# DJjjjhao/FIRA-ICSE

Measured on AMD Instinct MI355X. Metric: training commits/sec (FIRA default config), higher is better.
Workload: dtype f32; 1 GPU; BASELINE configs[1]: FIRA training step (fwd+bwd+Adam, dropout 0.1/0.2), batch 32 commits/GPU, fp32, 650-node graphs (mean nnz 1066/graph), vocab 24650; global_batch=32, parallelism=dp1

## Files before the change

fira_icse_amd/_lib.py:

```python
from __future__ import annotations

import ctypes as C
import os

HERE = os.path.dirname(os.path.abspath(__file__))
LIB_PATH = os.environ.get("FIRA_HIP_LIB") or os.path.join(HERE, "libfira_hip.so")


class FiraError(RuntimeError):
    pass


class Dims(C.Structure):
    _fields_ = [("sou_len", C.c_int32), ("sub_len", C.c_int32), ("ast_len", C.c_int32), ("tar_len", C.c_int32),
                ("d_model", C.c_int32), ("n_head", C.c_int32), ("n_layer", C.c_int32), ("vocab", C.c_int32),
                ("ast_vocab", C.c_int32), ("d_ff", C.c_int32)]


class Batch(C.Structure):
    _fields_ = [("B", C.c_int32), ("nnz", C.c_int32), ("sou", C.c_void_p), ("tar", C.c_void_p), ("mark", C.c_void_p),
                ("ast_change", C.c_void_p), ("tar_label", C.c_void_p), ("sub_token", C.c_void_p),
                ("n_nodes", C.c_int32), ("node_rows", C.c_void_p), ("rowptr", C.c_void_p), ("col", C.c_void_p),
                ("val", C.c_void_p), ("n_code", C.c_int32), ("code_rows", C.c_void_p), ("code_mark", C.c_void_p),
                ("n_mem", C.c_int32), ("mem_rows", C.c_void_p), ("mem_dst", C.c_void_p), ("head_rows", C.c_void_p),
# ... 59 lines not shown
    "fira_combination_block_bwd": (_I, [_P, _I, _P, _P, _P, _P, _P, _P, _P, _P, _P, _I, _P, _P, _P, _P, _P, _P, _I, _P, _F, _U64, _U32, _U32, _I]),
    "fira_combination_block_bwd_part_floats": (_I, []),
    "fira_embed_gather_fwd": (_I, [_P, _I, _I, _P, _P, _P, _P, _I, _I]),
    "fira_embed_gather_bwd": (_I, [_P, _I, _I, _P, _P, _P, _I, _I, _I]),
    "fira_combination_fwd": (_I, [_P, _I, _P, _P, _P, _P, _F, _U64, _U32]),
    "fira_combination_bwd": (_I, [_P, _I, _P, _P, _P, _P, _P, _P, _F, _U64, _U32]),
    "fira_add_layernorm_fwd": (_I, [_P, _I, _P, _P, _P, _P, _P, _P, _F, _U64, _U32]),
    "fira_linear_presum_f32": (_I, [_P, _I, _I, _P, _I, _P, _P, _P, _P, _F, _U64, _U32]),
    "fira_ln_linear_f32": (_I, [_P, _I, _I, _P, _I, _P, _P, _P, _I, _I, _P, _P, _P, _P]),
    "fira_ln_bwd_linear_f32": (_I, [_P, _I, _I, _P, _P, _P, _P, _P, _P, _P, _P, _P, _P, _P, _P, _F, _U64, _U32]),
    "fira_linear_layernorm_bf16_fwd": (_I, [_P, _I, _P, _I, _P, _I, _P, _P, _P, _P, _P, _P, _P, _F, _U64, _U32]),
    "fira_add_layernorm_bwd": (_I, [_P, _I, _P, _P, _P, _P, _P, _P, _P, _P, _F, _U64, _U32]),
    "fira_dropout_mask": (_I, [_P, _U64, _U32, _L, _F, _P]),
    "fira_colsum_f32": (_I, [_P, _I, _I, _P, _I, _P]),
    "fira_attention_fwd": (_I, [_P, _I, _I, _I, _I, _P, _I, _P, _I, _P, _I, _P, _I, _I, _P, _I]),
    "fira_attention_bwd": (_I, [_P, _I, _I, _I, _I, _P, _I, _P, _I, _P, _I, _P, _I, _I, _P, _I, _P, _I,
                                _P, _I, _P, _I, _P, _I]),
    "fira_attention_fwd_ex": (_I, [_P, _I, _I, _I, _I, _P, _I, _P, _I, _P, _I, _P, _I, _I, _P, _I, _P, _I, _I, _P]),
    "fira_attention_bwd_ex": (_I, [_P, _I, _I, _I, _I, _P, _I, _P, _I, _P, _I, _P, _I, _I, _P, _I, _P, _I,
                                   _P, _I, _P, _I, _P, _I, _P, _I, _I, _P]),
    "fira_decode_attention": (_I, [_P, _I, _I, _I, _P, _I, _P, _I, _P, _I, _P, _P, _I, _I, _I, _I, _P, _P, _I, _P, _P, _P]),
    "fira_copy_score_fwd": (_I, [_P, _I, _I, _I, _P, _P, _P, _P, _P]),
    "fira_copy_score_bwd": (_I, [_P, _I, _I, _I, _P, _P, _P, _P, _P, _P, _P, _P]),
    "fira_head_loss": (_I, [_P, _I, _I, _I, _I, _P, _P, _I, _P, _P, _P, _P, _P, _P, _P, _I]),
    "fira_adam_step": (_I, [_P, _L, _P, _P, _P, _P, _F, _F, _F, _F, _I, _P]),
    "fira_adam_step_mb": (_I, [_P, _L, _P, _P, _P, _P, _P, _F, _F, _F, _F, _I, _P, _P]),
    "fira_inv_count": (_I, [_P, _P, _P]),
    "fira_adam_step_count": (_I, [_P, _L, _P, _P, _P, _P, _F, _F, _F, _F, _I, _P]),
    "fira_pack_stats": (_I, [_P, _P, _P, _P]),
    "fira_debug_chain": (_I, [_P, _I, _I, _P]),
    "fira_train_fwd_bwd": (_I, [_P, _DP, _BP, _P, _P, _P, _Z, _OP, _P, _P, _P]),
    "fira_train_step": (_I, [_P, _DP, _BP, _P, _P, _P, _Z, _OP, _P, _P, C.POINTER(AdamOpts)]),
    "fira_gemm_wgrad_panel": (_I, [_P, _I, _I, _I, _I, _P, _I, _P, _I, _P, _I, _P, _P, _Z]),
    "fira_ffn_fwd": (_I, [_P, _I, _I] + [_P] * 11 + [_F, _U64, _U32, _I]),
    "fira_ffn_bwd": (_I, [_P, _I, _I] + [_P] * 17 + [_F, _U64, _U32, _I]),
    "fira_head_topk": (_I, [_P, _I, _I, _I, _P, _P, _P, _P, _I, _P, _P, _I]),
    "fira_train_step_rows": (_I, [_P, _DP, _BP, _P, _P, _P, _Z, _OP, _P, _P, C.POINTER(AdamOpts), _P]),
    "fira_adam_rows_sync": (_I, [_P, _DP, _P, C.POINTER(AdamOpts), _P]),
    "fira_adam_rows_catchup": (_I, [_P, _DP, _P, C.POINTER(AdamOpts), _P, _I, _P, _I]),
    "fira_adam_rows_step": (_I, [_P, _DP, _P, _P, C.POINTER(AdamOpts), _P, _P, _P, _I]),
    "fira_train_step_begin_rows": (_I, [_P, _DP, _BP, _P, _P, _P, _Z, _OP, _P, _P, _P, C.POINTER(AdamOpts), _P]),
    "fira_train_step_end_rows": (_I, [_P, _P, C.POINTER(AdamOpts), _P, _P, _P]),
    "fira_grad_sqsum_scratch_bytes": (_Z, []),
    "fira_grad_sqsum": (_I, [_P, _L, _P, _P, _I, _P]),
    "fira_clip_finish": (_I, [_P, _P, _I, _P, _P, _F]),
    "fira_adam_step_clip": (_I, [_P, _L, _P, _P, _P, _P, _F, _F, _F, _F, _I, _P, _P, _P]),
# ... 109 lines not shown
```

fira_icse_amd/csrc/copyhead.hip:

```cpp
#include "engine.h"
#include "adam_rows.h"
#include <stdlib.h>
#include "epilogue.h"
#include "decode_row.h"

namespace fira {

constexpr int T_MAX = 32;

__device__ __forceinline__ float tanh_fast(float x) {
    const float e = __expf(2.0f * x);
    return 1.0f - __fdividef(2.0f, 1.0f + e);
}

__global__ __launch_bounds__(256) void copy_score_fwd_kernel(int T, int S, const float* __restrict__ src,
                                                             const float* __restrict__ tgt,
                                                             const float* __restrict__ w,
                                                             const float* __restrict__ bias,
                                                             float* __restrict__ score, int qpk,
                                                             const int32_t* __restrict__ mem_valid, int slots,
                                                             const int32_t* __restrict__ tar_label, int V,
                                                             const int32_t* __restrict__ t_off) {
    __shared__ __attribute__((aligned(16))) float sm_tgt[T_MAX * FIRA_D];
    __shared__ unsigned sm_mask;
// ... 13 lines not shown
    const float4 w4 = *reinterpret_cast<const float4*>(w + lane * 4);
    const float c = bias[0];
    const int j_end = min(S, (int)(blockIdx.x + 1) * slots);
    for (int j = blockIdx.x * slots + wave; j < j_end; j += 4) {
        if (mv && mv[j] == 0) {
            if (lane < Tb) score[((size_t)tb + lane) * S + j] = 0.f;
            continue;
        }
        const float4 s4 = *reinterpret_cast<const float4*>(src + ((size_t)b * S + j) * FIRA_D + lane * 4);
        for (int t = 0; t < Tb; ++t) {
            if (!((mask >> t) & 1u)) continue;
            const float4 x = *reinterpret_cast<const float4*>(&sm_tgt[t * FIRA_D + lane * 4]);
            float a = w4.x * tanh_fast(s4.x + x.x);
            a = fmaf(w4.y, tanh_fast(s4.y + x.y), a);
            a = fmaf(w4.z, tanh_fast(s4.z + x.z), a);
            a = fmaf(w4.w, tanh_fast(s4.w + x.w), a);
            a = wave_sum(a);
            if (lane == 0) score[((size_t)tb + t) * S + j] = a + c;
        }
    }
}

constexpr int COPY_KA = 8;
__global__ __launch_bounds__(256) void copy_score_bwd_kernel(int T, int S, const float* __restrict__ src,
                                                             const float* __restrict__ tgt,
                                                             const float* __restrict__ w,
                                                             const float* __restrict__ dscore,
                                                             float* __restrict__ dsrc, float* __restrict__ dtgt,
                                                             float* __restrict__ dw, float* __restrict__ dbias,
                                                             const int32_t* __restrict__ mem_valid, int slots,
                                                             float* __restrict__ part,
                                                             const int32_t* __restrict__ t_off) {
    constexpr int SLOTS_MAX = 16, SPW = SLOTS_MAX / 4;
    __shared__ __attribute__((aligned(16))) float sm_tgt[COPY_KA * FIRA_D];
    __shared__ float sm_dt[COPY_KA * FIRA_D];
    __shared__ float sm_dw[FIRA_D + 1];
    __shared__ float sm_g[T_MAX * SLOTS_MAX];
    __shared__ unsigned sm_mask;
    const int b = blockIdx.y, t0 = threadIdx.x, lane = t0 & 63, wave = t0 >> 6;
    const int j0 = blockIdx.x * slots, j_end = min(S, j0 + slots);
    const int tb = t_off ? t_off[b] : b * T;
    const int Tb = t_off ? t_off[b + 1] - tb : T;
    if (t0 == 0) sm_mask = 0u;
    __syncthreads();
    for (int i = t0; i < Tb * slots; i += 256) {
        const int t = i / slots, j = j0 + i % slots;
        float g = 0.f;
        if (j < j_end && !(mem_valid && mem_valid[(size_t)b * S + j] == 0)) g = dscore[((size_t)tb + t) * S + j];
        sm_g[t * SLOTS_MAX + i % slots] = g;
        if (g != 0.f) atomicOr(&sm_mask, 1u << t);
    }
    for (int i = t0; i < FIRA_D + 1; i += 256) sm_dw[i] = 0.f;
    __syncthreads();
    const unsigned mask = sm_mask;
    float* const my_part = part ? part + ((size_t)blockIdx.y * gridDim.x + blockIdx.x) * COPY_PART_STRIDE : nullptr;
    if (mask == 0u) {
        for (int j = j0 + wave; j < j_end; j += 4)
            *reinterpret_cast<float4*>(dsrc + ((size_t)b * S + j) * FIRA_D + lane * 4) = make_float4(0.f, 0.f, 0.f, 0.f);
        if (my_part)
            for (int i = t0; i < FIRA_D + 1; i += 256) my_part[i] = 0.f;
        return;
    }
    const float4 w4 = *reinterpret_cast<const float4*>(w + lane * 4);
    const float wv[4] = {w4.x, w4.y, w4.z, w4.w};
    float4 s4[SPW];
    float ds[SPW][4];
    bool live[SPW];
#pragma unroll
    for (int q = 0; q < SPW; ++q) {
        const int j = j0 + wave + 4 * q;
        live[q] = j < j_end && !(mem_valid && mem_valid[(size_t)b * S + min(j, S - 1)] == 0);
        s4[q] = live[q] ? *reinterpret_cast<const float4*>(src + ((size_t)b * S + j) * FIRA_D + lane * 4)
                        : make_float4(0.f, 0.f, 0.f, 0.f);
#pragma unroll
        for (int e = 0; e < 4; ++e) ds[q][e] = 0.f;
    }
    float dwa[4] = {0.f, 0.f, 0.f, 0.f};
    float dba = 0.f;
    unsigned rem = mask;
    while (rem) {
        int tl[COPY_KA], nk = 0;
#pragma unroll
        for (int k = 0; k < COPY_KA; ++k) {
            tl[k] = 0;
            if (rem) { tl[k] = __ffs(rem) - 1; rem &= rem - 1; nk = k + 1; }
        }
#pragma unroll
        for (int k = 0; k < COPY_KA; ++k)
            if (k < nk && t0 < FIRA_D / 4)
                reinterpret_cast<float4*>(sm_tgt)[k * (FIRA_D / 4) + t0] =
                    reinterpret_cast<const float4*>(tgt + ((size_t)tb + tl[k]) * FIRA_D)[t0];
        for (int i = t0; i < COPY_KA * FIRA_D; i += 256) sm_dt[i] = 0.f;
        __syncthreads();
        float dt[COPY_KA][4];
#pragma unroll
        for (int k = 0; k < COPY_KA; ++k)
#pragma unroll
            for (int e = 0; e < 4; ++e) dt[k][e] = 0.f;
#pragma unroll
        for (int q = 0; q < SPW; ++q) {
            if (!live[q]) continue;
            const int jj = wave + 4 * q;
#pragma unroll
            for (int k = 0; k < COPY_KA; ++k) {
                if (k < nk) {
                    const float g = sm_g[tl[k] * SLOTS_MAX + jj];
                    const float4 x = *reinterpret_cast<const float4*>(&sm_tgt[k * FIRA_D + lane * 4]);
                    const float th[4] = {tanh_fast(s4[q].x + x.x), tanh_fast(s4[q].y + x.y), tanh_fast(s4[q].z + x.z),
                                         tanh_fast(s4[q].w + x.w)};
#pragma unroll
                    for (int e = 0; e < 4; ++e) {
                        const float u = g * wv[e] * (1.f - th[e] * th[e]);
                        ds[q][e] += u;
                        dt[k][e] += u;
                        dwa[e] = fmaf(g, th[e], dwa[e]);
                    }
                    dba += g;
                }
            }
        }
#pragma unroll
        for (int k = 0; k < COPY_KA; ++k)
            if (k < nk) {
#pragma unroll
                for (int e = 0; e < 4; ++e) atomicAdd(&sm_dt[k * FIRA_D + lane * 4 + e], dt[k][e]);
            }
        __syncthreads();
#pragma unroll
        for (int k = 0; k < COPY_KA; ++k)
            if (k < nk) unsafeAtomicAdd(&dtgt[((size_t)tb + tl[k]) * FIRA_D + t0], sm_dt[k * FIRA_D + t0]);
        __syncthreads();
    }
#pragma unroll
    for (int q = 0; q < SPW; ++q) {
        const int j = j0 + wave + 4 * q;
        if (j < j_end)
            *reinterpret_cast<float4*>(dsrc + ((size_t)b * S + j) * FIRA_D + lane * 4) = make_float4(ds[q][0], ds[q][1], ds[q][2], ds[q][3]);
    }
#pragma unroll
    for (int e = 0; e < 4; ++e) atomicAdd(&sm_dw[lane * 4 + e], dwa[e]);
    if (lane == 0) atomicAdd(&sm_dw[FIRA_D], dba);
    __syncthreads();
    if (my_part) {
        for (int i = t0; i < FIRA_D + 1; i += 256) my_part[i] = sm_dw[i];
        return;
    }
    for (int i = t0; i < FIRA_D; i += 256) unsafeAtomicAdd(&dw[i], sm_dw[i]);
    if (t0 == 0) unsafeAtomicAdd(dbias, sm_dw[FIRA_D]);
}

__device__ __forceinline__ float block_max(float v, float* sm) {
    v = wave_max(v);
    __syncthreads();
    if ((threadIdx.x & 63) == 0) sm[threadIdx.x >> 6] = v;
    __syncthreads();
    return fmaxf(fmaxf(sm[0], sm[1]), fmaxf(sm[2], sm[3]));
}
__device__ __forceinline__ float block_sum(float v, float* sm) {
    v = wave_sum(v);
    __syncthreads();
    if ((threadIdx.x & 63) == 0) sm[threadIdx.x >> 6] = v;
    __syncthreads();
    return (sm[0] + sm[1]) + (sm[2] + sm[3]);
}
__device__ __forceinline__ void block_argmax(float& v, int& idx, float* smv, int* smi) {
#pragma unroll
    for (int o = 32; o > 0; o >>= 1) {
        const float ov = __shfl_xor(v, o, 64);
        const int oi = __shfl_xor(idx, o, 64);
        if (ov > v || (ov == v && oi < idx)) { v = ov; idx = oi; }
    }
// ... 554 lines not shown
    else
    hipLaunchKernelGGL(decode_dist_kernel, dim3(R), dim3(256), 0, s, V, S, logits, ldl, score, mem_valid, qpk,
                       gate_logits, dist, best_id, best_p);
    FIRA_CHECK_LAUNCH("decode_dist");
    return 0;
}

int copy_score_fwd_ex(hipStream_t s, int B, int T, int S, const float* src, const float* tgt, const float* w,
                      const float* bias, float* score, int qpk, const int32_t* mem_valid, const int32_t* tar_label,
                      int V, const int32_t* t_off) {
    ProfScope prof(s, PROF_COPY, 0.0);
    if (B <= 0) return 0;
    FIRA_REQUIRE(T <= T_MAX && qpk >= 1, "copy_score_fwd: T=%d > %d", T, T_MAX);
    const int slots = 8;
    hipLaunchKernelGGL(copy_score_fwd_kernel, dim3(cdiv(S, slots), B), dim3(256), 0, s, T, S, src, tgt, w, bias, score,
                       qpk, mem_valid, slots, tar_label, V, t_off);
    FIRA_CHECK_LAUNCH("copy_score_fwd");
    return 0;
}
int copy_score_fwd(hipStream_t s, int B, int T, int S, const float* src, const float* tgt, const float* w,
                   const float* bias, float* score) {
    return copy_score_fwd_ex(s, B, T, S, src, tgt, w, bias, score, 1, nullptr, nullptr, 0, nullptr);
}
int copy_score_bwd_blocks(int B, int S) { return B > 0 ? cdiv(S, 16) * B : 0; }
int copy_score_bwd_ex(hipStream_t s, int B, int T, int S, const float* src, const float* tgt, const float* w,
                      const float* dscore, float* dsrc, float* dtgt, float* dw, float* dbias, const int32_t* mem_valid,
                      float* part, const int32_t* t_off) {
    ProfScope prof(s, PROF_COPY, 0.0);
    if (B <= 0) return 0;
    FIRA_REQUIRE(T <= T_MAX, "copy_score_bwd: T=%d > %d", T, T_MAX);
    const int slots = 16;
    hipLaunchKernelGGL(copy_score_bwd_kernel, dim3(cdiv(S, slots), B), dim3(256), 0, s, T, S, src, tgt, w, dscore, dsrc,
                       dtgt, dw, dbias, mem_valid, slots, part, t_off);
    FIRA_CHECK_LAUNCH("copy_score_bwd");
    return 0;
}
int copy_score_bwd(hipStream_t s, int B, int T, int S, const float* src, const float* tgt, const float* w,
                   const float* dscore, float* dsrc, float* dtgt, float* dw, float* dbias) {
    return copy_score_bwd_ex(s, B, T, S, src, tgt, w, dscore, dsrc, dtgt, dw, dbias, nullptr, nullptr, nullptr);
}
int head_loss(hipStream_t s, int BT, int T, int V, int S, const int32_t* compact_row, float* logits, int ldl,
              float* score, const int32_t* mem_valid, float* gate_logits, const int32_t* tar_label, float* loss_sum,
              int32_t* n_tok, int32_t* argmax_out, int want_grad, const int32_t* row_bt) {
    ProfScope prof(s, PROF_HEAD, 0.0);
    if (BT <= 0) return 0;
    const bool reg = (V % 2 == 0) && (V / 2 <= 256 * HL_PAIRS) && (ldl % 2 == 0) && ((uintptr_t)logits % 8 == 0);
    if (reg && !argmax_out)
        hipLaunchKernelGGL(head_loss_train_kernel, dim3(BT), dim3(256), 0, s, T, V, S, compact_row, logits, ldl, score,
                           mem_valid, gate_logits, tar_label, loss_sum, n_tok, want_grad, row_bt);
    else if (reg)
        hipLaunchKernelGGL(head_loss_kernel<true>, dim3(BT), dim3(256), 0, s, T, V, S, compact_row, logits, ldl, score,
                           mem_valid, gate_logits, tar_label, loss_sum, n_tok, argmax_out, want_grad, row_bt);
    else
        hipLaunchKernelGGL(head_loss_kernel<false>, dim3(BT), dim3(256), 0, s, T, V, S, compact_row, logits, ldl, score,
                           mem_valid, gate_logits, tar_label, loss_sum, n_tok, argmax_out, want_grad, row_bt);
    FIRA_CHECK_LAUNCH("head_loss");
    return 0;
}
int adam_step(hipStream_t s, int64_t n, float* p, const float* g, float* m, float* v, float lr, float beta1,
              float beta2, float eps, int step, const float* scale_ptr, int scale_is_count) {
    ProfScope prof(s, PROF_ADAM, 0.0);
    if (n <= 0) return 0;
// ... 62 lines not shown
    const int grid = std::min(cdiv(total, 4), 256 * 8);
    hipLaunchKernelGGL(adam_rows_catchup_kernel, dim3(grid), dim3(256), 0, s, tb, l, beta1, beta2, eps, to,
                       adam_rows_hist(lr, beta1, beta2, to), 0.0f);
    FIRA_CHECK_LAUNCH("adam_rows_catchup");
    return 0;
}
int inv_count(hipStream_t s, const int32_t* n_tok, float* out) {
    hipLaunchKernelGGL(inv_count_kernel, dim3(1), dim3(1), 0, s, n_tok, out);
    FIRA_CHECK_LAUNCH("inv_count");
    return 0;
}

}

extern "C" {
int fira_copy_score_fwd(void* stream, int B, int T, int S, const float* src, const float* tgt, const float* w,
                        const float* bias, float* score) {
    return fira::copy_score_fwd((hipStream_t)stream, B, T, S, src, tgt, w, bias, score);
}
int fira_copy_score_bwd(void* stream, int B, int T, int S, const float* src, const float* tgt, const float* w,
                        const float* dscore, float* dsrc, float* dtgt, float* dw, float* dbias) {
    return fira::copy_score_bwd((hipStream_t)stream, B, T, S, src, tgt, w, dscore, dsrc, dtgt, dw, dbias);
}
int fira_head_loss(void* stream, int BT, int T, int V, int S, const int32_t* compact_row, float* logits, int ldl,
                   float* score, const int32_t* mem_valid, float* gate_logits, const int32_t* tar_label,
                   float* loss_sum, int32_t* n_tok, int32_t* argmax_out, int want_grad) {
    return fira::head_loss((hipStream_t)stream, BT, T, V, S, compact_row, logits, ldl, score, mem_valid, gate_logits,
                           tar_label, loss_sum, n_tok, argmax_out, want_grad);
}
int fira_adam_step_mb(void* stream, int64_t n, float* p, const float* g0, const float* g1, float* m, float* v, float lr,
                      float beta1, float beta2, float eps, int step, const int32_t* n_tok0, const int32_t* n_tok1) {
    FIRA_REQUIRE(p && g0 && m && v && n_tok0 && step >= 1, "fira_adam_step_mb: bad argument");
    return fira::adam_step_mb((hipStream_t)stream, n, p, g0, g1, m, v, lr, beta1, beta2, eps, step, n_tok0, n_tok1);
}
int fira_inv_count(void* stream, const int32_t* n_tok, float* out) {
    return fira::inv_count((hipStream_t)stream, n_tok, out);
}
int fira_adam_step(void* stream, int64_t n, float* p, const float* g, float* m, float* v, float lr, float beta1,
                   float beta2, float eps, int step, const float* inv_scale_ntok) {
    return fira::adam_step((hipStream_t)stream, n, p, g, m, v, lr, beta1, beta2, eps, step, inv_scale_ntok, 0);
}
int fira_adam_step_count(void* stream, int64_t n, float* p, const float* g, float* m, float* v, float lr, float beta1,
                         float beta2, float eps, int step, const float* count) {
    FIRA_REQUIRE(p && g && m && v && count && step >= 1, "fira_adam_step_count: bad argument");
    return fira::adam_step((hipStream_t)stream, n, p, g, m, v, lr, beta1, beta2, eps, step, count, 1);
}
// ... 8 lines not shown
```

fira_icse_amd/csrc/engine.h:

```cpp
#pragma once
#include "common.h"
#include <string>
#include <vector>

namespace fira {

int gemm_f32(hipStream_t s, int tA, int tB, int M, int N, int K, const float* A, int lda, const float* B, int ldb,
             float* C, int ldc, const float* bias, int flags, int splitk);
int gemm_f32_ex(hipStream_t s, int tA, int tB, int M, int N, int K, const float* A, int lda, const float* B, int ldb,
                float* C, int ldc, const float* bias, int flags, int splitk, float* colsum,
                const int32_t* c_rows = nullptr, const float* relu_mask = nullptr);
int gemm_bf16_ex(hipStream_t s, int tA, int tB, int M, int N, int K, const float* A, int lda, const float* B, int ldb,
                 float* C, int ldc, const float* bias, int flags, int splitk, float* colsum,
                 const int32_t* c_rows = nullptr, const float* relu_mask = nullptr);
struct ShadowEntry { int64_t offset; int rows, cols, pitch_t; int64_t offset_t; };
constexpr int SHADOW_MAX = 64;
struct ShadowTable {
    int n = 0;
    int64_t wbt_elems = 0;
    int tile_start[SHADOW_MAX + 1] = {0};
    ShadowEntry e[SHADOW_MAX];
};
int weight_shadows(hipStream_t s, const ShadowTable& tab, const float* P, uint16_t* Wb, uint16_t* WbT);
int gemm_bf16_wb_ex(hipStream_t s, int M, int N, int K, const float* A, int lda, const uint16_t* Bb, int ldb, float* C,
// ... 160 lines not shown
                     const float* V, int ldv, const int32_t* key_valid, float* O, int ldo, int kb, int kvb, int qpk,
                     const float* Knew = nullptr, const float* Vnew = nullptr, int ldn = 0, float* Kc_out = nullptr,
                     float* Vc_out = nullptr, const int32_t* k_off = nullptr);
int decode_self_block(hipStream_t s, int BR, int Tk, int T, const float* qkv, float* Kc, float* Vc, const int32_t* hist,
                      const float* WoT, const float* bo, const float* xres, const float* gamma, const float* beta,
                      const float* WqT, const float* bq, float* xa, float* qc);
int decode_attention_kv16(hipStream_t s, int BR, int H, int Tk, const float* Q, int ldq, const uint16_t* K, int ldk,
                          const uint16_t* V, int ldv, const int32_t* key_valid, float* O, int ldo, int kb, int kvb, int qpk,
                          const int32_t* k_off = nullptr);
int rows_to_bf16(hipStream_t s, int64_t n, const float* in, uint16_t* out);
int rows_from_bf16(hipStream_t s, int64_t n, const uint16_t* in, float* out);
int attention_bwd(hipStream_t s, int B, int H, int Tq, int Tk, const float* Q, int ldq, const float* K, int ldk,
                  const float* V, int ldv, const int32_t* key_valid, int causal, int q_pos0, const float* O, int ldo,
                  const float* dO, int lddo, float* dQ, int lddq, float* dK, int lddk, float* dV, int lddv,
                  const int32_t* q_off = nullptr, int self_kv = 0, int bf16 = 0, const int32_t* k_off = nullptr);
int copy_score_fwd(hipStream_t s, int B, int T, int S, const float* src, const float* tgt, const float* w,
                   const float* bias, float* score);
int copy_score_fwd_ex(hipStream_t s, int B, int T, int S, const float* src, const float* tgt, const float* w,
                      const float* bias, float* score, int qpk, const int32_t* mem_valid,
                      const int32_t* tar_label = nullptr, int V = 0,
                      const int32_t* t_off = nullptr);
int copy_score_bwd_ex(hipStream_t s, int B, int T, int S, const float* src, const float* tgt, const float* w,
                      const float* dscore, float* dsrc, float* dtgt, float* dw, float* dbias, const int32_t* mem_valid,
                      float* part = nullptr, const int32_t* t_off = nullptr);
int copy_score_bwd_blocks(int B, int S);
constexpr int COPY_PART_STRIDE = 264;
int decode_dist(hipStream_t s, int R, int V, int S, const float* logits, int ldl, const float* score,
                const int32_t* mem_valid, int qpk, const float* gate_logits, float* dist, int32_t* best_id,
                float* best_p, const float* x = nullptr, const float* wp = nullptr, const float* bp = nullptr);
int inv_count(hipStream_t s, const int32_t* n_tok, float* out);
int sample_dist(hipStream_t s, int R, int n_sample, int V, int S, const float* logits, int ldl, const float* score,
                const int32_t* mem_valid, const float* x, const float* wp, const float* bp, int T, int step,
                const int32_t* key, const uint64_t* seed_dev, float temperature, int top_k, float top_p, float* dist,
                int32_t* best_id, float* best_p);
int score_dist(hipStream_t s, int R, int n_cand, int V, int L, int S, const float* logits, int ldl, const float* score,
               const int32_t* mem_valid, const float* x, const float* wp, const float* bp, const int32_t* target,
               const int32_t* label, const int32_t* sou, const int32_t* sub, float* dist, float* p_word, float* p_entry,
               int32_t* entry, float* copy_share, float* p_label, int32_t* top_id, float* logp_word, float* logp_entry,
               float* logp_label);
int row_topk(hipStream_t s, int R, int V, int k, const float* logits, int ldl, int32_t* ids, float* vals);
int copy_score_bwd(hipStream_t s, int B, int T, int S, const float* src, const float* tgt, const float* w,
                   const float* dscore, float* dsrc, float* dtgt, float* dw, float* dbias);
int head_loss(hipStream_t s, int BT, int T, int V, int S, const int32_t* compact_row, float* logits, int ldl,
              float* score, const int32_t* mem_valid, float* gate_logits, const int32_t* tar_label, float* loss_sum,
              int32_t* n_tok, int32_t* argmax_out, int want_grad,
              const int32_t* row_bt = nullptr);
int adam_step(hipStream_t s, int64_t n, float* p, const float* g, float* m, float* v, float lr, float beta1,
              float beta2, float eps, int step, const float* scale_ptr, int scale_is_count = 0);
// ... 72 lines not shown
```

fira_icse_amd/csrc/engine.hip:

```cpp
#include "engine.h"
#include <hip/hip_ext.h>
#include "epilogue.h"
#include <stdlib.h>
#include <map>
#include <mutex>

namespace fira {

static int64_t shadow_wbt_elems(const Layout& L);

struct Arena {
    char* base;
    size_t used = 0;
    explicit Arena(void* b) : base((char*)b) {}
    template <typename T>
    T* get(size_t n) {
        size_t bytes = (n * sizeof(T) + 255) / 256 * 256;
        T* p = base ? (T*)(base + used) : nullptr;
        used += bytes;
        return p;
    }
    float* f(size_t n) { return get<float>(n); }
};

// ... 27 lines not shown
    std::vector<DecGrad> decg;
    float *vtab_all, *H, *mem, *mem_c, *src_c, *x0, *kv_all, *src, *tgt, *score, *gate, *dec_c, *logits;
    float *W21, *c21, *rsum;
    float *W21t;
    uint16_t *W21x = nullptr, *W21tx = nullptr;
    uint16_t *WcX = nullptr, *WcTX = nullptr;
    uint16_t* WkvX = nullptr;
    float* WkvT = nullptr;
    uint16_t* WkvTX = nullptr;
    uint16_t* WoutTX = nullptr;
    uint16_t *xh_planes = nullptr;
    float *WcT;
    float *dW21, *dc21;
    float *inv_ntok;
    float *dXa, *dXb, *dNB2, *dCB_a, *dvtab_all;
    float *zero_beg = nullptr, *zero_end = nullptr;
    uint16_t *wb = nullptr, *wbt = nullptr;
    uint16_t *w21b = nullptr, *w21bt = nullptr;
    float* red_buf = nullptr;
    size_t red_cap = 0;
    float* panel_scratch = nullptr;
    size_t panel_floats = 0;
    float *dmem_c, *dsrc, *dsrc_c, *dtgt, *dkv_all, *ddec, *ddec_c, *dT_a, *dT_c;

    size_t build(void* ws, const fira_dims& d, int B_, bool training) {
        Arena a(ws);
        B = B_; L = d.sou_len; S = d.sub_len; A = d.ast_len; T = d.tar_len; V = d.vocab; nl = d.n_layer; F = d.d_ff;
        N = L + S + A;
        NB = B * N; CB = B * L; MB = B * (L + S); TB = B * T;
        ldl = (V + 63) / 64 * 64;
        const size_t D = FIRA_D;
        pos_code = a.f((size_t)L * D);
        pos_tar = a.f((size_t)T * D);
        mem_valid = a.get<int32_t>((size_t)MB);
        tar_valid = a.get<int32_t>((size_t)TB);
        compact_row = a.get<int32_t>((size_t)TB);
        iota = a.get<int32_t>((size_t)TB);
        row_bt = a.get<int32_t>((size_t)TB);
        rows_c = a.get<int32_t>((size_t)TB);
        code_slot = a.get<int32_t>((size_t)NB);
        mem_slot = a.get<int32_t>((size_t)NB);
        mem_off = a.get<int32_t>((size_t)B + 1);
        mem_valid_c = a.get<int32_t>((size_t)MB);
        inv_ntok = a.f(64);
        {
            const Layout* lay = get_layout(&d);
// ... 39 lines not shown
            e.st_a = a.f((size_t)TB * 2); e.x_a = a.f((size_t)TB * D); e.qc = a.f((size_t)TB * D);
            e.ao2 = a.f((size_t)TB * D); e.s_c = a.f((size_t)TB * D); e.st_c = a.f((size_t)TB * 2);
            e.x_c = a.f((size_t)TB * D); e.h = a.f((size_t)TB * F); e.s_f = a.f((size_t)TB * D);
            e.st_f = a.f((size_t)TB * 2); e.x_f = a.f((size_t)TB * D);
        }
        src = a.f((size_t)MB * D); tgt = a.f((size_t)TB * D);
        score = a.f((size_t)TB * (L + S)); gate = a.f((size_t)TB * 2);
        dec_c = a.f((size_t)TB * D); logits = a.f((size_t)TB * ldl);
        if (training) {
            dXa = a.f((size_t)NB * D); dXb = a.f((size_t)NB * D); dNB2 = a.f((size_t)NB * D);
            dCB_a = a.f((size_t)CB * D);
            red_cap = (size_t)nl * ((size_t)cdiv(NB, 16) * 4 * D + (size_t)cdiv(CB, 16) * 2 * D)
                    + (size_t)3 * nl * cdiv(TB, 16) * 2 * D
                    + (size_t)nl * std::max((size_t)cdiv(CB, 16) * 4 * D, (size_t)comb_fused_bwd_parts() * 6 * D + 64)
                    + (size_t)cdiv(L + S, 16) * B * COPY_PART_STRIDE + 4096;
            red_buf = a.f(red_cap);
            panel_floats = (size_t)320 * 256 * 256;
            panel_scratch = a.f(panel_floats);
            zero_beg = (float*)a.get<char>(0);
            dvtab_all = a.f((size_t)4 * nl * D);
            dW21 = a.f((size_t)nl * D * D + (size_t)nl * D); dc21 = dW21 + (size_t)nl * D * D;
            dtgt = a.f((size_t)TB * D);
            ddec_c = a.f((size_t)TB * D);
            zero_end = (float*)a.get<char>(0);
            dmem_c = a.f((size_t)MB * D); dsrc = a.f((size_t)MB * D); dsrc_c = a.f((size_t)MB * D);
            dkv_all = a.f((size_t)MB * kvp);
            ddec = a.f((size_t)TB * D);
            dT_a = a.f((size_t)TB * D); dT_c = a.f((size_t)TB * D);
            encg.resize(nl);
            decg.resize(nl);
            for (int l = 0; l < nl; ++l) {
                EncGrad& g = encg[l];
                g.dY2 = a.f((size_t)NB * D); g.dYc = a.f((size_t)CB * D);
                g.dqk = a.f((size_t)CB * 2 * D);
                DecGrad& h = decg[l];
                h.dYf = a.f((size_t)TB * D); h.dh = a.f((size_t)TB * F); h.dYc = a.f((size_t)TB * D);
                h.dq = a.f((size_t)TB * D); h.dYs = a.f((size_t)TB * D); h.dqkv = a.f((size_t)TB * 3 * D);
            }
        }
        return a.used;
    }
};

#define TRY(x)                 \
    do {                       \
        if (int e__ = (x)) return e__; \
    } while (0)
// ... 863 lines not shown
    const bool so = side_on();
    hipStream_t ss = so ? side().aux : s;
    hipEvent_t ev_dfc = nullptr;
    if (c.ev_zero) TRY(main_wait(s, c.ev_zero, __LINE__));
    else TRY(zero(s, p.zero_beg, (size_t)((char*)p.zero_end - (char*)p.zero_beg)));
    if (R > 0) {
        if (so) TRY(aux_fork(s));
        if (c.wout_planes) TRY(dgrad_x3_splitk(ss, R, p.V, p.logits, p.ldl, p.WoutTX, p.ddec_c, D, g_dtype == 1));
        else
        TRY(gemm_any(ss, 0, 0, R, D, p.V, p.logits, p.ldl, c.P + L.wout, D, p.ddec_c, D, nullptr, FIRA_GEMM_ACCUM, 0,
                        nullptr));
        if (so) TRY(side_mark(&ev_dfc));
    }
    if (R > 0)
        TRY(linear_wgrad(s, R, p.V, D, p.logits, p.ldl, (c.rows != nullptr && rows == c.rows) ? p.dec_c : dec, D, G + L.wout,
                         G + L.bout, PANEL_VOCAB));
    if (g_dtype == 0) TRY(rank2_rows(s, c.Td, p.gate, c.P + L.wp, p.ddec));
    else TRY(linear_dgrad(s, c.Td, 2, D, p.gate, 2, c.P + L.wp, p.ddec, D, false));
    TRY(linear_wgrad_grouped(s, c.Td, 2, D, p.gate, 2, dec, D, G + L.wp, G + L.bp));
    {
        const int nb = copy_score_bwd_blocks(p.B, Sm);
        float* part = red().alloc((size_t)nb * COPY_PART_STRIDE);
        TRY(copy_score_bwd_ex(s, p.B, p.T, Sm, p.src, p.tgt, c.P + L.wres, p.score, p.dsrc, p.dtgt, G + L.wres, G + L.bres,
                              p.mem_valid, part, c.dec_off));
        if (part) {
            red().add(G + L.wres, part, D, nb, COPY_PART_STRIDE);
            red().add(G + L.bres, part + D, 1, nb, COPY_PART_STRIDE);
        }
    }
    TRY(linear_dgrad(s, c.Td, D, D, p.dtgt, D, c.P + L.wt, p.ddec, D, true));
    TRY(linear_wgrad_grouped(s, c.Td, D, D, p.dtgt, D, dec, D, G + L.wt, nullptr));
    TRY(rows_move(s, 0, Mc, D, p.dsrc_c, p.dsrc, bt.mem_dst, nullptr));
    if (so) TRY(aux_fork(s));
    TRY(linear_dgrad(ss, Mc, D, D, p.dsrc_c, D, c.P + L.ws, p.dmem_c, D, false));
    TRY(linear_wgrad_grouped(s, Mc, D, D, p.dsrc_c, D, p.mem_c, D, G + L.ws, nullptr, 8));
    if (R > 0) {
        if (ev_dfc) TRY(main_wait(s, ev_dfc, __LINE__));
        TRY(rows_scatter_add_idx(s, R, p.ddec_c, p.ddec, rows));
    }

    float *bx = p.ddec, *by = p.dT_a, *bz = p.dT_c;
    constexpr int DEC_WGRAD_EVERY = 3;
    const int dec_every = p.nl % DEC_WGRAD_EVERY != 0 ? 0 : DEC_WGRAD_EVERY;
    {
    ProfScope prof_region(s, PROF_DEC_REGION, 0.0);
    TRY(lanes_fork(c));
    auto aux_fork_all = [&]() -> int { return c.n_lanes > 1 ? lanes_fork_to(c, side().aux) : aux_fork(s); };
// ... 934 lines not shown
```

fira_icse_amd/ops.py:

```python
from __future__ import annotations

import dataclasses

import torch

from . import _lib
from ._lib import check, cur_stream, ptr


def _f32(t):
    assert t.is_cuda and t.dtype == torch.float32 and t.is_contiguous(), "expected a contiguous fp32 CUDA tensor"
    return t


def _i32(t):
    assert t.is_cuda and t.dtype == torch.int32 and t.is_contiguous(), "expected a contiguous int32 CUDA tensor"
    return t


def gemm(A, B, *, transA=False, transB=True, bias=None, relu=False, out=None, accumulate=False, splitk=1,
         tile=0, dtype="f32"):
    for t in (A, B):
        assert t.is_cuda and t.dtype == torch.float32 and t.dim() == 2 and t.stride(1) == 1
    M, K = (A.shape[1], A.shape[0]) if transA else A.shape
# ... 338 lines not shown

def copy_score_fwd(src, tgt, w, bias):
    B, S, _ = src.shape
    T = tgt.shape[1]
    score = torch.empty((B, T, S), dtype=torch.float32, device=src.device)
    check(_lib.lib().fira_copy_score_fwd(cur_stream(), B, T, S, ptr(_f32(src)), ptr(_f32(tgt)), ptr(_f32(w)),
                                         ptr(_f32(bias)), ptr(score)), "fira_copy_score_fwd")
    return score


def copy_score_bwd(src, tgt, w, dscore):
    B, S, _ = src.shape
    T = tgt.shape[1]
    dsrc = torch.empty_like(src)
    dtgt = torch.zeros_like(tgt)
    dw = torch.zeros(256, dtype=torch.float32, device=src.device)
    db = torch.zeros(1, dtype=torch.float32, device=src.device)
    check(_lib.lib().fira_copy_score_bwd(cur_stream(), B, T, S, ptr(_f32(src)), ptr(_f32(tgt)), ptr(_f32(w)),
                                         ptr(_f32(dscore)), ptr(dsrc), ptr(dtgt), ptr(dw), ptr(db)),
          "fira_copy_score_bwd")
    return dsrc, dtgt, dw, db


def head_loss(logits, score, mem_valid, gate_logits, tar_label, V, compact_row=None, want_grad=True, argmax=False):
    B, T = tar_label.shape
    S = score.shape[-1]
    loss = torch.zeros(1, dtype=torch.float32, device=logits.device)
    ntok = torch.zeros(1, dtype=torch.int32, device=logits.device)
    ids = torch.empty((B, T), dtype=torch.int32, device=logits.device) if argmax else None
    check(_lib.lib().fira_head_loss(cur_stream(), B * T, T, V, S, ptr(compact_row), ptr(_f32(logits)),
                                    logits.stride(0), ptr(_f32(score)), ptr(_i32(mem_valid)), ptr(_f32(gate_logits)),
                                    ptr(_i32(tar_label)), ptr(loss), ptr(ntok), ptr(ids), int(want_grad)),
          "fira_head_loss")
    return loss, ntok, ids


def adam_step(p, g, m, v, lr, step, beta1=0.9, beta2=0.999, eps=1e-8, inv_scale=None):
    check(_lib.lib().fira_adam_step(cur_stream(), p.numel(), ptr(_f32(p)), ptr(_f32(g)), ptr(_f32(m)), ptr(_f32(v)),
                                    lr, beta1, beta2, eps, step, ptr(inv_scale)), "fira_adam_step")


def adam_step_count(p, g, m, v, lr, step, count, beta1=0.9, beta2=0.999, eps=1e-8):
    check(_lib.lib().fira_adam_step_count(cur_stream(), p.numel(), ptr(_f32(p)), ptr(_f32(g)), ptr(_f32(m)), ptr(_f32(v)),
                                          lr, beta1, beta2, eps, step, ptr(_f32(count))), "fira_adam_step_count")


# ... 177 lines not shown
```

include/fira_hip.h:

```cpp
#ifndef FIRA_HIP_H
#define FIRA_HIP_H

#include <stddef.h>
#include <stdint.h>

#ifdef __cplusplus
extern "C" {
#endif

#define FIRA_ABI_VERSION 10

typedef struct fira_dims {
    int32_t sou_len;
    int32_t sub_len;
    int32_t ast_len;
    int32_t tar_len;
    int32_t d_model;
    int32_t n_head;
    int32_t n_layer;
    int32_t vocab;
    int32_t ast_vocab;
    int32_t d_ff;
} fira_dims;

// ... 157 lines not shown
                       const float* K, int ldk, const float* V, int ldv, const int32_t* key_valid,
                       int causal, int q_pos0, const float* O, int ldo, const float* dO, int lddo,
                       float* dQ, int lddq, float* dK, int lddk, float* dV, int lddv);
int fira_attention_fwd_ex(void* stream, int B, int H, int Tq, int Tk, const float* Q, int ldq,
                          const float* K, int ldk, const float* V, int ldv, const int32_t* key_valid,
                          int causal, int q_pos0, float* O, int ldo, const int32_t* q_off, int self_kv, int dtype,
                          const int32_t* k_off);
int fira_attention_bwd_ex(void* stream, int B, int H, int Tq, int Tk, const float* Q, int ldq,
                          const float* K, int ldk, const float* V, int ldv, const int32_t* key_valid,
                          int causal, int q_pos0, const float* O, int ldo, const float* dO, int lddo,
                          float* dQ, int lddq, float* dK, int lddk, float* dV, int lddv,
                          const int32_t* q_off, int self_kv, int dtype, const int32_t* k_off);

int fira_decode_attention(void* stream, int BR, int H, int Tk, const float* Q, int ldq, const float* K, int ldk,
                          const float* V, int ldv, const int32_t* key_valid, float* O, int ldo, int kb, int kvb, int qpk,
                          const float* Knew, const float* Vnew, int ldn, float* Kc_out, float* Vc_out,
                          const int32_t* k_off);

int fira_copy_score_fwd(void* stream, int B, int T, int S, const float* src, const float* tgt,
                        const float* w, const float* bias, float* score);
int fira_copy_score_bwd(void* stream, int B, int T, int S, const float* src, const float* tgt,
                        const float* w, const float* dscore, float* dsrc , float* dtgt ,
                        float* dw , float* dbias );

int fira_head_loss(void* stream, int BT, int T, int V, int S, const int32_t* compact_row,
                   float* logits, int ldl, float* score , const int32_t* mem_valid ,
                   float* gate_logits , const int32_t* tar_label ,
                   float* loss_sum, int32_t* n_tok, int32_t* argmax_out, int want_grad);

int fira_adam_step(void* stream, int64_t n, float* p, const float* g, float* m, float* v,
                   float lr, float beta1, float beta2, float eps, int step, const float* inv_scale_ntok);
int fira_adam_step_mb(void* stream, int64_t n, float* p, const float* g0, const float* g1, float* m, float* v,
                      float lr, float beta1, float beta2, float eps, int step, const int32_t* n_tok0,
                      const int32_t* n_tok1);
int fira_adam_step_count(void* stream, int64_t n, float* p, const float* g, float* m, float* v,
                         float lr, float beta1, float beta2, float eps, int step, const float* count);
int fira_pack_stats(void* stream, const float* loss_sum, const int32_t* n_tok, float* out2);
int fira_inv_count(void* stream, const int32_t* n_tok, float* out);

int fira_debug_chain(void* stream, int n, int mode, float* scratch);


int fira_train_fwd_bwd(void* stream, const fira_dims* d, const fira_batch* batch, const float* params,
                       float* grads, void* workspace, size_t workspace_bytes, const fira_train_opts* opts,
                       float* loss_sum, int32_t* n_tok, void* mid_event);

// ... 150 lines not shown
```

Before: 13880 commits/s.

## Replace copy-score dtgt global atomics with per-block partials and last-block reduction

The copy-score backward kernel used to add each block's target gradient into dtgt with global float atomics. It now writes per-block partial rows plus a per-block t-mask into scratch. A per-batch atomic counter picks the last block to finish, and that block sums the partial rows that are live under the mask. The tanh derivative is also recomputed algebraically from a single exp and reciprocal. The aim is to remove atomic contention, at the cost of scratch memory traffic and a serial reduction in one block per batch.

```diff
diff --git a/fira_icse_amd/_lib.py b/fira_icse_amd/_lib.py
--- a/fira_icse_amd/_lib.py
+++ b/fira_icse_amd/_lib.py
@@ -105,6 +105,8 @@
     "fira_decode_attention": (_I, [_P, _I, _I, _I, _P, _I, _P, _I, _P, _I, _P, _P, _I, _I, _I, _I, _P, _P, _I, _P, _P, _P]),
     "fira_copy_score_fwd": (_I, [_P, _I, _I, _I, _P, _P, _P, _P, _P]),
     "fira_copy_score_bwd": (_I, [_P, _I, _I, _I, _P, _P, _P, _P, _P, _P, _P, _P]),
+    "fira_copy_score_bwd_scratch": (_L, [_I, _I, _I, _I]),
+    "fira_copy_score_bwd_ex": (_I, [_P, _I, _I, _I, _P, _P, _P, _P, _P, _P, _P, _P, _P, _P, _P]),
     "fira_head_loss": (_I, [_P, _I, _I, _I, _I, _P, _P, _I, _P, _P, _P, _P, _P, _P, _P, _I]),
     "fira_adam_step": (_I, [_P, _L, _P, _P, _P, _P, _F, _F, _F, _F, _I, _P]),
     "fira_adam_step_mb": (_I, [_P, _L, _P, _P, _P, _P, _P, _F, _F, _F, _F, _I, _P, _P]),
diff --git a/fira_icse_amd/csrc/copyhead.hip b/fira_icse_amd/csrc/copyhead.hip
--- a/fira_icse_amd/csrc/copyhead.hip
+++ b/fira_icse_amd/csrc/copyhead.hip
@@ -59,45 +59,49 @@
 }
 
 constexpr int COPY_KA = 8;
+constexpr int COPY_SLOTS = 16;
+template <bool PARTS>
 __global__ __launch_bounds__(256) void copy_score_bwd_kernel(int T, int S, const float* __restrict__ src,
                                                              const float* __restrict__ tgt,
                                                              const float* __restrict__ w,
                                                              const float* __restrict__ dscore,
                                                              float* __restrict__ dsrc, float* __restrict__ dtgt,
                                                              float* __restrict__ dw, float* __restrict__ dbias,
-                                                             const int32_t* __restrict__ mem_valid, int slots,
+                                                             const int32_t* __restrict__ mem_valid,
                                                              float* __restrict__ part,
-                                                             const int32_t* __restrict__ t_off) {
-    constexpr int SLOTS_MAX = 16, SPW = SLOTS_MAX / 4;
+                                                             const int32_t* __restrict__ t_off,
+                                                             float* dt_part, int32_t* dt_cnt) {
+    constexpr int slots = COPY_SLOTS, SPW = COPY_SLOTS / 4;
     __shared__ __attribute__((aligned(16))) float sm_tgt[COPY_KA * FIRA_D];
-    __shared__ float sm_dt[COPY_KA * FIRA_D];
+    __shared__ __attribute__((aligned(16))) float sm_dt[COPY_KA * FIRA_D];
     __shared__ float sm_dw[FIRA_D + 1];
-    __shared__ float sm_g[T_MAX * SLOTS_MAX];
+    __shared__ float sm_g[T_MAX * COPY_SLOTS];
     __shared__ unsigned sm_mask;
     const int b = blockIdx.y, t0 = threadIdx.x, lane = t0 & 63, wave = t0 >> 6;
     const int j0 = blockIdx.x * slots, j_end = min(S, j0 + slots);
     const int tb = t_off ? t_off[b] : b * T;
     const int Tb = t_off ? t_off[b + 1] - tb : T;
+    const size_t blk = (size_t)blockIdx.y * gridDim.x + blockIdx.x;
     if (t0 == 0) sm_mask = 0u;
     __syncthreads();
     for (int i = t0; i < Tb * slots; i += 256) {
         const int t = i / slots, j = j0 + i % slots;
         float g = 0.f;
         if (j < j_end && !(mem_valid && mem_valid[(size_t)b * S + j] == 0)) g = dscore[((size_t)tb + t) * S + j];
-        sm_g[t * SLOTS_MAX + i % slots] = g;
+        sm_g[t * COPY_SLOTS + i % slots] = g;
         if (g != 0.f) atomicOr(&sm_mask, 1u << t);
     }
     for (int i = t0; i < FIRA_D + 1; i += 256) sm_dw[i] = 0.f;
     __syncthreads();
-    const unsigned mask = sm_mask;
-    float* const my_part = part ? part + ((size_t)blockIdx.y * gridDim.x + blockIdx.x) * COPY_PART_STRIDE : nullptr;
+    const unsigned mask = __builtin_amdgcn_readfirstlane(sm_mask);
+    float* const my_part = part ? part + blk * COPY_PART_STRIDE : nullptr;
     if (mask == 0u) {
         for (int j = j0 + wave; j < j_end; j += 4)
             *reinterpret_cast<float4*>(dsrc + ((size_t)b * S + j) * FIRA_D + lane * 4) = make_float4(0.f, 0.f, 0.f, 0.f);
         if (my_part)
             for (int i = t0; i < FIRA_D + 1; i += 256) my_part[i] = 0.f;
-        return;
-    }
+        if (!PARTS) return;
+    } else {
     const float4 w4 = *reinterpret_cast<const float4*>(w + lane * 4);
     const float wv[4] = {w4.x, w4.y, w4.z, w4.w};
     float4 s4[SPW];
@@ -138,19 +142,23 @@
         for (int q = 0; q < SPW; ++q) {
             if (!live[q]) continue;
             const int jj = wave + 4 * q;
+            const float sv[4] = {s4[q].x, s4[q].y, s4[q].z, s4[q].w};
 #pragma unroll
             for (int k = 0; k < COPY_KA; ++k) {
                 if (k < nk) {
-                    const float g = sm_g[tl[k] * SLOTS_MAX + jj];
+                    const float g = sm_g[tl[k] * COPY_SLOTS + jj];
                     const float4 x = *reinterpret_cast<const float4*>(&sm_tgt[k * FIRA_D + lane * 4]);
-                    const float th[4] = {tanh_fast(s4[q].x + x.x), tanh_fast(s4[q].y + x.y), tanh_fast(s4[q].z + x.z),
-                                         tanh_fast(s4[q].w + x.w)};
+                    const float xv[4] = {x.x, x.y, x.z, x.w};
+                    const float g4 = 4.0f * g;
+                    const float gw[4] = {g4 * wv[0], g4 * wv[1], g4 * wv[2], g4 * wv[3]};
 #pragma unroll
                     for (int e = 0; e < 4; ++e) {
-                        const float u = g * wv[e] * (1.f - th[e] * th[e]);
+                        const float ex = __expf(fminf(2.0f * (sv[e] + xv[e]), 80.0f));
+                        const float r = __builtin_amdgcn_rcpf(1.0f + ex);
+                        const float u = gw[e] * ((ex * r) * r);
                         ds[q][e] += u;
                         dt[k][e] += u;
-                        dwa[e] = fmaf(g, th[e], dwa[e]);
+                        dwa[e] = fmaf(g, fmaf(-2.0f, r, 1.0f), dwa[e]);
                     }
                     dba += g;
                 }
@@ -163,9 +171,19 @@
                 for (int e = 0; e < 4; ++e) atomicAdd(&sm_dt[k * FIRA_D + lane * 4 + e], dt[k][e]);
             }
         __syncthreads();
-#pragma unroll
-        for (int k = 0; k < COPY_KA; ++k)
-            if (k < nk) unsafeAtomicAdd(&dtgt[((size_t)tb + tl[k]) * FIRA_D + t0], sm_dt[k * FIRA_D + t0]);
+        if (PARTS) {
+#pragma unroll
+            for (int k = 0; k < COPY_KA; ++k)
+                if (k < nk && (k & 3) == wave) {
+                    const float4 v = *reinterpret_cast<const float4*>(&sm_dt[k * FIRA_D + lane * 4]);
+                    const rsrc_t rp = buf_rsrc(dt_part + (blk * T + tl[k]) * FIRA_D, FIRA_D * 4u);
+                    __builtin_amdgcn_raw_buffer_store_b128(__builtin_bit_cast(u32v4_t, v), rp, lane * 16, 0, 16);
+                }
+        } else {
+#pragma unroll
+            for (int k = 0; k < COPY_KA; ++k)
+                if (k < nk) unsafeAtomicAdd(&dtgt[((size_t)tb + tl[k]) * FIRA_D + t0], sm_dt[k * FIRA_D + t0]);
+        }
         __syncthreads();
     }
 #pragma unroll
@@ -180,10 +198,62 @@
     __syncthreads();
     if (my_part) {
         for (int i = t0; i < FIRA_D + 1; i += 256) my_part[i] = sm_dw[i];
-        return;
-    }
-    for (int i = t0; i < FIRA_D; i += 256) unsafeAtomicAdd(&dw[i], sm_dw[i]);
-    if (t0 == 0) unsafeAtomicAdd(dbias, sm_dw[FIRA_D]);
+    } else {
+        for (int i = t0; i < FIRA_D; i += 256) unsafeAtomicAdd(&dw[i], sm_dw[i]);
+        if (t0 == 0) unsafeAtomicAdd(dbias, sm_dw[FIRA_D]);
+    }
+    if (!PARTS) return;
+    }
+    if (PARTS) {
+        unsigned* const masks = reinterpret_cast<unsigned*>(dt_part + (size_t)gridDim.y * gridDim.x * T * FIRA_D);
+        const int gx = gridDim.x;
+        if (t0 == 0) __hip_atomic_store(&masks[blk], mask, __ATOMIC_RELAXED, __HIP_MEMORY_SCOPE_AGENT);
+        asm volatile("s_waitcnt vmcnt(0)" ::: "memory");
+        __syncthreads();
+        if (t0 == 0)
+            sm_mask = __hip_atomic_fetch_add(&dt_cnt[b], 1, __ATOMIC_RELAXED, __HIP_MEMORY_SCOPE_AGENT) == gx - 1 ? 1u : 0u;
+        __syncthreads();
+        if (sm_mask == 0u) return;
+        if (t0 == 0) {
+            __hip_atomic_store(&dt_cnt[b], 0, __ATOMIC_RELAXED, __HIP_MEMORY_SCOPE_AGENT);
+            __builtin_amdgcn_fence(__ATOMIC_ACQUIRE, "agent");
+            asm volatile("s_waitcnt vmcnt(0)" ::: "memory");
+        }
+        __syncthreads();
+        unsigned* const sm_tm = reinterpret_cast<unsigned*>(sm_g);
+        constexpr int COPY_TM = T_MAX * COPY_SLOTS;
+        const unsigned* const cmask = masks + (size_t)b * gx;
+        for (int xc = 0; xc < gx; xc += COPY_TM) {
+            const int nx = min(COPY_TM, gx - xc);
+            __syncthreads();
+            for (int i = t0; i < nx; i += 256) sm_tm[i] = cmask[xc + i];
+            __syncthreads();
+            for (int t = wave; t < Tb; t += 4) {
+                const float* const prow = dt_part + (((size_t)b * gx + xc) * T + t) * FIRA_D + lane * 4;
+                float4 acc = make_float4(0.f, 0.f, 0.f, 0.f);
+                bool hit = false;
+                for (int x0 = 0; x0 < nx; x0 += 8) {
+                    float4 v[8];
+#pragma unroll
+                    for (int u = 0; u < 8; ++u) {
+                        const int xx = x0 + u;
+                        const bool on = xx < nx && ((sm_tm[min(xx, nx - 1)] >> t) & 1u);
+                        v[u] = make_float4(0.f, 0.f, 0.f, 0.f);
+                        if (on) v[u] = *reinterpret_cast<const float4*>(prow + (size_t)xx * T * FIRA_D);
+                        hit |= on;
+                    }
+#pragma unroll
+                    for (int u = 0; u < 8; ++u) { acc.x += v[u].x; acc.y += v[u].y; acc.z += v[u].z; acc.w += v[u].w; }
+                }
+                if (hit) {
+                    float4* const d = reinterpret_cast<float4*>(dtgt + ((size_t)tb + t) * FIRA_D + lane * 4);
+                    float4 o = *d;
+                    o.x += acc.x; o.y += acc.y; o.z += acc.z; o.w += acc.w;
+                    *d = o;
+                }
+            }
+        }
+    }
 }
 
 __device__ __forceinline__ float block_max(float v, float* sm) {
@@ -784,22 +854,31 @@
                    const float* bias, float* score) {
     return copy_score_fwd_ex(s, B, T, S, src, tgt, w, bias, score, 1, nullptr, nullptr, 0, nullptr);
 }
-int copy_score_bwd_blocks(int B, int S) { return B > 0 ? cdiv(S, 16) * B : 0; }
+int copy_score_bwd_blocks(int B, int S) { return B > 0 ? cdiv(S, COPY_SLOTS) * B : 0; }
+size_t copy_score_bwd_dt_floats(int B, int T, int S) {
+    const size_t nb = (size_t)copy_score_bwd_blocks(B, S);
+    return nb * T * FIRA_D + (nb + 63) / 64 * 64;
+}
 int copy_score_bwd_ex(hipStream_t s, int B, int T, int S, const float* src, const float* tgt, const float* w,
                       const float* dscore, float* dsrc, float* dtgt, float* dw, float* dbias, const int32_t* mem_valid,
-                      float* part, const int32_t* t_off) {
+                      float* part, const int32_t* t_off, float* dt_part, int32_t* dt_cnt) {
     ProfScope prof(s, PROF_COPY, 0.0);
     if (B <= 0) return 0;
     FIRA_REQUIRE(T <= T_MAX, "copy_score_bwd: T=%d > %d", T, T_MAX);
-    const int slots = 16;
-    hipLaunchKernelGGL(copy_score_bwd_kernel, dim3(cdiv(S, slots), B), dim3(256), 0, s, T, S, src, tgt, w, dscore, dsrc,
-                       dtgt, dw, dbias, mem_valid, slots, part, t_off);
+    FIRA_REQUIRE((dt_part == nullptr) == (dt_cnt == nullptr), "copy_score_bwd: partial dtgt rows need their counters");
+    const dim3 grid(cdiv(S, COPY_SLOTS), B);
+    if (dt_part)
+        hipLaunchKernelGGL(copy_score_bwd_kernel<true>, grid, dim3(256), 0, s, T, S, src, tgt, w, dscore, dsrc, dtgt, dw,
+                           dbias, mem_valid, part, t_off, dt_part, dt_cnt);
+    else
+        hipLaunchKernelGGL(copy_score_bwd_kernel<false>, grid, dim3(256), 0, s, T, S, src, tgt, w, dscore, dsrc, dtgt, dw,
+                           dbias, mem_valid, part, t_off, dt_part, dt_cnt);
     FIRA_CHECK_LAUNCH("copy_score_bwd");
     return 0;
 }
 int copy_score_bwd(hipStream_t s, int B, int T, int S, const float* src, const float* tgt, const float* w,
                    const float* dscore, float* dsrc, float* dtgt, float* dw, float* dbias) {
-    return copy_score_bwd_ex(s, B, T, S, src, tgt, w, dscore, dsrc, dtgt, dw, dbias, nullptr, nullptr, nullptr);
+    return copy_score_bwd_ex(s, B, T, S, src, tgt, w, dscore, dsrc, dtgt, dw, dbias, nullptr, nullptr, nullptr, nullptr, nullptr);
 }
 int head_loss(hipStream_t s, int BT, int T, int V, int S, const int32_t* compact_row, float* logits, int ldl,
               float* score, const int32_t* mem_valid, float* gate_logits, const int32_t* tar_label, float* loss_sum,
@@ -908,6 +987,18 @@
                         const float* dscore, float* dsrc, float* dtgt, float* dw, float* dbias) {
     return fira::copy_score_bwd((hipStream_t)stream, B, T, S, src, tgt, w, dscore, dsrc, dtgt, dw, dbias);
 }
+int64_t fira_copy_score_bwd_scratch(int B, int T, int S, int which) {
+    if (which == 0) return (int64_t)fira::copy_score_bwd_blocks(B, S) * fira::COPY_PART_STRIDE;
+    if (which == 1) return (int64_t)fira::copy_score_bwd_dt_floats(B, T, S);
+    return fira::COPY_PART_STRIDE;
+}
+int fira_copy_score_bwd_ex(void* stream, int B, int T, int S, const float* src, const float* tgt, const float* w,
+                           const float* dscore, float* dsrc, float* dtgt, const int32_t* mem_valid, const int32_t* t_off,
+                           float* part, float* dt_part, int32_t* dt_cnt) {
+    FIRA_REQUIRE(src && tgt && w && dscore && dsrc && dtgt && part && dt_part && dt_cnt, "fira_copy_score_bwd_ex: null pointer argument");
+    return fira::copy_score_bwd_ex((hipStream_t)stream, B, T, S, src, tgt, w, dscore, dsrc, dtgt, nullptr, nullptr, mem_valid,
+                                   part, t_off, dt_part, dt_cnt);
+}
 int fira_head_loss(void* stream, int BT, int T, int V, int S, const int32_t* compact_row, float* logits, int ldl,
                    float* score, const int32_t* mem_valid, float* gate_logits, const int32_t* tar_label,
                    float* loss_sum, int32_t* n_tok, int32_t* argmax_out, int want_grad) {
diff --git a/fira_icse_amd/csrc/engine.h b/fira_icse_amd/csrc/engine.h
--- a/fira_icse_amd/csrc/engine.h
+++ b/fira_icse_amd/csrc/engine.h
@@ -206,8 +206,10 @@
                       const int32_t* t_off = nullptr);
 int copy_score_bwd_ex(hipStream_t s, int B, int T, int S, const float* src, const float* tgt, const float* w,
                       const float* dscore, float* dsrc, float* dtgt, float* dw, float* dbias, const int32_t* mem_valid,
-                      float* part = nullptr, const int32_t* t_off = nullptr);
+                      float* part = nullptr, const int32_t* t_off = nullptr, float* dt_part = nullptr,
+                      int32_t* dt_cnt = nullptr);
 int copy_score_bwd_blocks(int B, int S);
+size_t copy_score_bwd_dt_floats(int B, int T, int S);
 constexpr int COPY_PART_STRIDE = 264;
 int decode_dist(hipStream_t s, int R, int V, int S, const float* logits, int ldl, const float* score,
                 const int32_t* mem_valid, int qpk, const float* gate_logits, float* dist, int32_t* best_id,
diff --git a/fira_icse_amd/csrc/engine.hip b/fira_icse_amd/csrc/engine.hip
--- a/fira_icse_amd/csrc/engine.hip
+++ b/fira_icse_amd/csrc/engine.hip
@@ -73,6 +73,8 @@
     float* panel_scratch = nullptr;
     size_t panel_floats = 0;
     float *dmem_c, *dsrc, *dsrc_c, *dtgt, *dkv_all, *ddec, *ddec_c, *dT_a, *dT_c;
+    float* copy_dt = nullptr;
+    int32_t* copy_cnt = nullptr;
 
     size_t build(void* ws, const fira_dims& d, int B_, bool training) {
         Arena a(ws);
@@ -158,7 +160,9 @@
             dW21 = a.f((size_t)nl * D * D + (size_t)nl * D); dc21 = dW21 + (size_t)nl * D * D;
             dtgt = a.f((size_t)TB * D);
             ddec_c = a.f((size_t)TB * D);
+            copy_cnt = a.get<int32_t>((size_t)B);
             zero_end = (float*)a.get<char>(0);
+            copy_dt = a.f(copy_score_bwd_dt_floats(B, T, L + S));
             dmem_c = a.f((size_t)MB * D); dsrc = a.f((size_t)MB * D); dsrc_c = a.f((size_t)MB * D);
             dkv_all = a.f((size_t)MB * kvp);
             ddec = a.f((size_t)TB * D);
@@ -1068,7 +1072,7 @@
         const int nb = copy_score_bwd_blocks(p.B, Sm);
         float* part = red().alloc((size_t)nb * COPY_PART_STRIDE);
         TRY(copy_score_bwd_ex(s, p.B, p.T, Sm, p.src, p.tgt, c.P + L.wres, p.score, p.dsrc, p.dtgt, G + L.wres, G + L.bres,
-                              p.mem_valid, part, c.dec_off));
+                              p.mem_valid, part, c.dec_off, p.copy_dt, p.copy_cnt));
         if (part) {
             red().add(G + L.wres, part, D, nb, COPY_PART_STRIDE);
             red().add(G + L.bres, part + D, 1, nb, COPY_PART_STRIDE);
diff --git a/fira_icse_amd/ops.py b/fira_icse_amd/ops.py
--- a/fira_icse_amd/ops.py
+++ b/fira_icse_amd/ops.py
@@ -384,6 +384,27 @@
     return dsrc, dtgt, dw, db
 
 
+def copy_score_bwd_scratch(B, T, S, device):
+    L = _lib.lib()
+    stride = L.fira_copy_score_bwd_scratch(B, T, S, 2)
+    part = torch.empty((L.fira_copy_score_bwd_scratch(B, T, S, 0) // stride, stride), dtype=torch.float32, device=device)
+    dt_part = torch.empty(L.fira_copy_score_bwd_scratch(B, T, S, 1), dtype=torch.float32, device=device)
+    dt_cnt = torch.zeros(B, dtype=torch.int32, device=device)
+    return part, dt_part, dt_cnt
+
+
+def copy_score_bwd_ex(src, tgt, w, dscore, dsrc, dtgt, scratch, mem_valid=None, t_off=None, T=None):
+    B, S, _ = src.shape
+    T = tgt.shape[1] if T is None else T
+    part, dt_part, dt_cnt = scratch
+    check(_lib.lib().fira_copy_score_bwd_ex(cur_stream(), B, T, S, ptr(_f32(src)), ptr(_f32(tgt)), ptr(_f32(w)),
+                                            ptr(_f32(dscore)), ptr(_f32(dsrc)), ptr(_f32(dtgt)),
+                                            ptr(_i32(mem_valid)) if mem_valid is not None else None,
+                                            ptr(_i32(t_off)) if t_off is not None else None, ptr(part), ptr(dt_part),
+                                            ptr(dt_cnt)), "fira_copy_score_bwd_ex")
+    return part
+
+
 def head_loss(logits, score, mem_valid, gate_logits, tar_label, V, compact_row=None, want_grad=True, argmax=False):
     B, T = tar_label.shape
     S = score.shape[-1]
diff --git a/include/fira_hip.h b/include/fira_hip.h
--- a/include/fira_hip.h
+++ b/include/fira_hip.h
@@ -203,6 +203,10 @@
 int fira_copy_score_bwd(void* stream, int B, int T, int S, const float* src, const float* tgt,
                         const float* w, const float* dscore, float* dsrc , float* dtgt ,
                         float* dw , float* dbias );
+int64_t fira_copy_score_bwd_scratch(int B, int T, int S, int which);
+int fira_copy_score_bwd_ex(void* stream, int B, int T, int S, const float* src, const float* tgt, const float* w,
+                           const float* dscore, float* dsrc , float* dtgt , const int32_t* mem_valid,
+                           const int32_t* t_off, float* part , float* dt_part, int32_t* dt_cnt);
 
 int fira_head_loss(void* stream, int BT, int T, int V, int S, const int32_t* compact_row,
                    float* logits, int ldl, float* score , const int32_t* mem_valid ,
```

Result: no change. 13770 commits/s (-0.8%).
